# arnold117/PrimeKG-RGCN-LinkPrediction

Measured on AMD Instinct MI355X. Metric: edges/sec per RGCN layer (fwd+bwd), PrimeKG 30.9k nodes/849k edges/3 rels, higher is better.
Workload: dtype f32; 1 GPU; C2: PrimeKG-shaped synthetic graph, 30926 nodes / 849456 edge columns / 3 relations, encoder 64->128->128, 2 layers fwd+bwd, full graph per step, dropout 0; parallelism=1 GPU, launch=hipGraph replay

## Files before the change

### include/rgcn_hip.h

```cpp
#ifndef RGCN_HIP_H
#define RGCN_HIP_H

#include <stddef.h>
#include <stdint.h>

#ifdef __cplusplus
extern "C" {
#endif

#define RGCN_ABI_VERSION 27

enum {
  RGCN_OK = 0,
  RGCN_ERR_ARG = -1,
  RGCN_ERR_RANGE = -2,
  RGCN_ERR_HIP = -3,
  RGCN_ERR_UNSUPPORTED = -4,
  RGCN_ERR_WORKSPACE = -5
};

int rgcn_abi_version(void);
const char* rgcn_strerror(int code);

typedef struct rgcn_graph rgcn_graph;

int rgcn_graph_create(const int64_t* edge_index, const int64_t* edge_type, int64_t num_edges,
                      int64_t num_nodes, int64_t num_relations, void* stream,
                      rgcn_graph** out);
int rgcn_graph_create_bipartite(const int64_t* key_node, const int64_t* other_node,
                                const int64_t* edge_type, int64_t num_edges, int64_t num_key_nodes,
                                int64_t num_other_nodes, int64_t num_relations,
                                const float* edge_weight, void* stream, rgcn_graph** out);
void rgcn_graph_destroy(rgcn_graph* g);

int64_t rgcn_graph_num_edges(const rgcn_graph* g);
int64_t rgcn_graph_num_nodes(const rgcn_graph* g);
int64_t rgcn_graph_num_relations(const rgcn_graph* g);
float rgcn_graph_weight_bound(const rgcn_graph* g, int transposed);
int rgcn_graph_num_levels(const rgcn_graph* g, int transposed);

const uint32_t* rgcn_graph_tile_mask(const rgcn_graph* g, int transposed, int64_t* num_row_tiles);

int rgcn_graph_arrays(const rgcn_graph* g, int transposed, const int32_t** rowptr,
                      const int32_t** col, const int64_t** perm, const float** val);
int rgcn_graph_export(const rgcn_graph* g, int transposed, int32_t* rowptr, int32_t* col,
                      int64_t* perm, float* val, void* stream);

int rgcn_graph_import(int64_t num_edges, int64_t num_nodes, int64_t num_relations,
                      const int32_t* rowptr, const int32_t* col, const int64_t* perm, const float* cnt,
                      const int32_t* rowptr_t, const int32_t* col_t, const int64_t* perm_t,
                      const float* w_t, void* stream, rgcn_graph** out);

typedef struct rgcn_slab_job {
  const float* slab;
// ... 215 lines not shown
```

### primekg_rgcn_linkprediction_amd/_lib.py

```python
from __future__ import annotations

import ctypes
import os
from ctypes import c_float, POINTER, c_char_p, c_int, c_int64, c_size_t, c_void_p

import torch

ABI_VERSION = 27
LIB_NAME = "librgcn_hip.so"
LIB_PATH = os.path.join(os.path.dirname(os.path.abspath(__file__)), LIB_NAME)

RGCN_OK = 0
RGCN_ERR_ARG = -1
RGCN_ERR_RANGE = -2
RGCN_ERR_HIP = -3
RGCN_ERR_UNSUPPORTED = -4
RGCN_ERR_WORKSPACE = -5

_P = c_void_p
_I64 = c_int64

class SlabJob(ctypes.Structure):
    _fields_ = [("slab", c_void_p), ("bias_part", c_void_p), ("splits", ctypes.c_int32), ("K1", ctypes.c_int32),
                ("Kc", ctypes.c_int32), ("N", ctypes.c_int32), ("grad_weight", c_void_p), ("grad_root", c_void_p),
# ... 21 lines not shown
                                      7: (True, 0), 8: (True, 0), 9: (False, 0)},
}


PROTOTYPES = {
    "rgcn_abi_version": (c_int, []),
    "rgcn_strerror": (c_char_p, [c_int]),
    "rgcn_graph_create": (c_int, [_P, _P, _I64, _I64, _I64, _P, POINTER(c_void_p)]),
    "rgcn_graph_create_bipartite": (c_int, [_P, _P, _P, _I64, _I64, _I64, _I64, _P, _P, POINTER(c_void_p)]),
    "rgcn_graph_destroy": (None, [c_void_p]),
    "rgcn_graph_num_edges": (_I64, [c_void_p]),
    "rgcn_graph_num_nodes": (_I64, [c_void_p]),
    "rgcn_graph_num_relations": (_I64, [c_void_p]),
    "rgcn_graph_num_levels": (c_int, [c_void_p, c_int]),
    "rgcn_graph_weight_bound": (c_float, [c_void_p, c_int]),
    "rgcn_graph_arrays": (c_int, [c_void_p, c_int, POINTER(c_void_p), POINTER(c_void_p),
                                  POINTER(c_void_p), POINTER(c_void_p)]),
    "rgcn_graph_export": (c_int, [c_void_p, c_int, _P, _P, _P, _P, _P]),
    "rgcn_graph_import": (c_int, [_I64, _I64, _I64, _P, _P, _P, _P, _P, _P, _P, _P, _P, POINTER(c_void_p)]),
    "rgcn_aggregate_workspace_bytes": (c_size_t, [c_void_p, c_int, _I64]),
    "rgcn_aggregate": (c_int, [c_void_p, c_int, _P, _I64, _P, _P, c_size_t, _P]),
    "rgcn_aggregate_f16": (c_int, [c_void_p, c_int, _P, _I64, _P, _P, c_size_t, _P]),
    "rgcn_aggregate_level": (c_int, [c_void_p, c_int, c_int, _P, _I64, _P, _P, c_size_t, _P, _P]),
    "rgcn_graph_tile_mask": (c_void_p, [c_void_p, c_int, POINTER(c_int64)]),
    "rgcn_transform_fwd": (c_int, [_P, _P, _P, _P, _P, c_int, _P, _I64, _I64, _I64, _I64, _P, _P]),
    "rgcn_transform_fwd_f16_workspace_bytes": (c_size_t, [_I64, _I64, _I64]),
    "rgcn_transform_fwd_f16": (c_int, [_P, _P, _P, _P, _P, c_int, _P, _I64, _I64, _I64, _I64, _P, _P, c_size_t, _P]),
    "rgcn_transform_bwd_input": (c_int, [_P, _P, _P, _P, _P, _P, _I64, _I64, _I64, _I64, _P, _P]),
    "rgcn_transform_bwd_params_workspace_bytes": (c_size_t, [_I64, _I64, _I64, _I64]),
    "rgcn_transform_bwd_params": (c_int, [_P, _P, _P, _P, _I64, _I64, _I64, _I64, _P, _P, _P, _P,
# ... 116 lines not shown
```

### primekg_rgcn_linkprediction_amd/csrc/rgcn_aggregate.hip

```cpp
#include <algorithm>
#include <cstdlib>
#include <type_traits>

#include <hip/hip_fp16.h>

#include "rgcn_common.h"
#include "rgcn_slab_reduce.h"
#include "rgcn_hub_finish.h"

namespace {

constexpr int kThreads = 256;
constexpr int kUnroll = RGCN_HEAD;
#ifndef RGCN_REDUCE_UNROLL
#define RGCN_REDUCE_UNROLL 16
#endif

__device__ inline float4 f4zero() { return make_float4(0.f, 0.f, 0.f, 0.f); }
__device__ inline float f4amax(const float4& a) { return fmaxf(fmaxf(fabsf(a.x), fabsf(a.y)), fmaxf(fabsf(a.z), fabsf(a.w))); }

__device__ inline void f4add(float4& a, const float4& b) { a.x += b.x; a.y += b.y; a.z += b.z; a.w += b.w; }
__device__ inline void f4fma(float4& a, const float4& b, float s) {
  a.x = fmaf(b.x, s, a.x); a.y = fmaf(b.y, s, a.y); a.z = fmaf(b.z, s, a.z); a.w = fmaf(b.w, s, a.w);
}
// ... 29 lines not shown
    }
  }
  __device__ inline void advance(int gl, const int32_t* __restrict__ col, const float* __restrict__ w) {
    pos += RGCN_HEAD;
    if (pos == len) {
      cur = nxt;
      curw = nxtw;
      pos = 0;
      len = G;
      nbase += G;
      fetch_next(gl, col, w);
    }
  }
};

template <int G, bool WEIGHTED>
__device__ inline void aggregate_block(
    const int bx, float4* red, const float* __restrict__ src, const rgcn_item* __restrict__ items, int64_t nitems,
    const int32_t* __restrict__ col, const float* __restrict__ w, const float* __restrict__ cnt,
    float* __restrict__ agg, float* __restrict__ partial, int d, const int32_t* __restrict__ head_col,
    const float* __restrict__ head_w, unsigned* __restrict__ amax_out) {
  const int64_t item_id = ((int64_t)bx * kThreads + threadIdx.x) / G;
  const int c4 = ((int)threadIdx.x % G + (int)blockIdx.y * G) * 4;
  if (item_id >= nitems) return;
  const unsigned seen = rgcn_amax_peek(amax_out);
  const bool live = c4 < d;
  const rgcn_item it = items[item_id];
  const bool has_packs = (items[(int64_t)bx * (kThreads / G)].flags & RGCN_ITEM_PACK) != 0;

  float4 acc = f4zero();
  if constexpr (G >= RGCN_HEAD) {
    const int gl = (int)threadIdx.x % G;
    IdWindow<G, WEIGHTED> win;
    win.init(item_id, gl, it, col, w, head_col, head_w);
    for (int e = it.begin; e < it.end; e += kUnroll) {
      int idx[kUnroll];
      float wt[kUnroll];
      float4 v[kUnroll];
      win.get(idx, wt);
#pragma unroll
      for (int u = 0; u < kUnroll; ++u) {
        v[u] = f4zero();
        if (live && idx[u] >= 0) v[u] = *reinterpret_cast<const float4*>(src + (size_t)idx[u] * d + c4);
      }
      win.advance(gl, col, w);
#pragma unroll
      for (int u = 0; u < kUnroll; ++u) {
        if (WEIGHTED) f4fma(acc, v[u], wt[u]);
        else f4add(acc, v[u]);
      }
    }
  } else if (live) {
    int idx_n[kUnroll];
    float wt_n[kUnroll];
#pragma unroll
    for (int u = 0; u < kUnroll; ++u) {
      idx_n[u] = head_col[item_id * kUnroll + u];
      wt_n[u] = WEIGHTED ? head_w[item_id * kUnroll + u] : 0.f;
    }
    for (int e = it.begin; e < it.end; e += kUnroll) {
      int idx[kUnroll];
      float wt[kUnroll];
      float4 v[kUnroll];
#pragma unroll
      for (int u = 0; u < kUnroll; ++u) {
        idx[u] = idx_n[u];
        wt[u] = wt_n[u];
      }
#pragma unroll
      for (int u = 0; u < kUnroll; ++u) {
        v[u] = f4zero();
        if (idx[u] >= 0) v[u] = *reinterpret_cast<const float4*>(src + (size_t)idx[u] * d + c4);
      }
#pragma unroll
      for (int u = 0; u < kUnroll; ++u) {
        const int en = e + kUnroll + u;
        const bool ok = en < it.end;
        idx_n[u] = ok ? col[en] : -1;
        wt_n[u] = (WEIGHTED && ok) ? w[en] : 0.f;
      }
#pragma unroll
      for (int u = 0; u < kUnroll; ++u) {
        if (WEIGHTED) f4fma(acc, v[u], wt[u]);
        else f4add(acc, v[u]);
      }
    }
  }
  if (has_packs) {
    red[threadIdx.x] = acc;
    __syncthreads();
    if (it.flags & (RGCN_ITEM_MEMBER | RGCN_ITEM_SKIP)) return;
    const int followers = (it.flags >> RGCN_ITEM_FOLLOW_SHIFT) & (RGCN_PACK - 1);
    for (int f = 1; f <= followers; ++f) f4add(acc, red[threadIdx.x + f * G]);
  }
  if (!live) return;
  float lmax = 0.f;
  if (it.flags & RGCN_ITEM_FINAL) {
    if (cnt) {
      const float c = cnt[it.dst];
      acc.x /= c; acc.y /= c; acc.z /= c; acc.w /= c;
    }
    *reinterpret_cast<float4*>(agg + (size_t)it.dst * d + c4) = acc;
    lmax = f4amax(acc);
  } else {
    *reinterpret_cast<float4*>(partial + (size_t)it.dst * d + c4) = acc;
  }
  if (amax_out) rgcn_amax_publish(amax_out, lmax, seen);
}

template <int G, bool WEIGHTED>
__global__ __launch_bounds__(kThreads) void k_aggregate(
    const float* __restrict__ src, const rgcn_item* __restrict__ items, int64_t nitems,
    const int32_t* __restrict__ col, const float* __restrict__ w, const float* __restrict__ cnt,
    float* __restrict__ agg, float* __restrict__ partial, int d, const int32_t* __restrict__ head_col,
    const float* __restrict__ head_w, const rgcn_slab_job job, int gather_blocks, unsigned* __restrict__ amax_out) {
  __shared__ float4 red[kThreads];
  if ((int)blockIdx.x >= gather_blocks) {
    rgcn_slab_reduce_block<RGCN_SLAB_OUTS, RGCN_SLAB_GROUPS>(job, (int64_t)blockIdx.x - gather_blocks, red);
    return;
  }
  aggregate_block<G, WEIGHTED>((int)blockIdx.x, red, src, items, nitems, col, w, cnt, agg, partial, d, head_col, head_w, amax_out);
}

template <int G, bool WEIGHTED>
__global__ __launch_bounds__(kThreads) void k_aggregate_h(
    const __half* __restrict__ src, const rgcn_item* __restrict__ items, int64_t nitems,
    const int32_t* __restrict__ col, const float* __restrict__ w, const float* __restrict__ cnt,
    float* __restrict__ agg, float* __restrict__ partial, int d, const int32_t* __restrict__ head_col,
    const float* __restrict__ head_w) {
  const int64_t item_id = ((int64_t)blockIdx.x * kThreads + threadIdx.x) / G;
  __shared__ float4 red[2 * kThreads];
  const int c8 = ((int)threadIdx.x % G + (int)blockIdx.y * G) * 8;
  if (item_id >= nitems) return;
  const bool live = c8 < d;
  const rgcn_item it = items[item_id];
  const bool has_packs = (items[(int64_t)blockIdx.x * (kThreads / G)].flags & RGCN_ITEM_PACK) != 0;

  float acc[8];
#pragma unroll
  for (int k = 0; k < 8; ++k) acc[k] = 0.f;
  auto accumulate = [&](const uint4 (&v)[kUnroll], const float (&wt)[kUnroll]) {
#pragma unroll
    for (int u = 0; u < kUnroll; ++u) {
      const __half2* h2 = reinterpret_cast<const __half2*>(&v[u]);
#pragma unroll
      for (int k = 0; k < 4; ++k) {
        const float2 f = __half22float2(h2[k]);
        if (WEIGHTED) {
          acc[2 * k] = fmaf(f.x, wt[u], acc[2 * k]);
          acc[2 * k + 1] = fmaf(f.y, wt[u], acc[2 * k + 1]);
        } else {
// ... 79 lines not shown
template <int G>
__global__ __launch_bounds__(kThreads) void k_reduce_partials(const rgcn_item* __restrict__ items,
                                                              const float* __restrict__ cnt,
                                                              float* __restrict__ agg, float* partial, int d,
                                                              unsigned* __restrict__ amax_out) {
  __shared__ float4 red[kThreads];
  const float lmax = rgcn_reduce_item<G>(items[blockIdx.x], cnt, agg, partial, d, (int)blockIdx.y * G, red);
  if (amax_out && (int)threadIdx.x < G && (((int)threadIdx.x + (int)blockIdx.y * G) * 4 < d) &&
      (items[blockIdx.x].flags & RGCN_ITEM_FINAL))
    rgcn_amax_publish(amax_out, lmax);
}

template <int G>
void launch_level(const rgcn_csr* c, int level, bool weighted, const float* x, const float* cnt, float* agg,
                  float* partial, int d, hipStream_t stream, const rgcn_slab_job* tail = nullptr,
                  unsigned* amax_out = nullptr) {
  const int64_t nitems = c->num_items[level];
  if (nitems == 0) return;
  const unsigned gy = (unsigned)ceil_div64(d, 4 * G);
  if (level == 0) {
    const unsigned gather_blocks = (unsigned)ceil_div64(nitems, kThreads / G);
    const rgcn_slab_job job = tail ? *tail : rgcn_slab_job{};
    dim3 grid(gather_blocks + (tail ? (unsigned)rgcn_slab_reduce_blocks(job) : 0u), gy);
    if (weighted)
      k_aggregate<G, true><<<grid, kThreads, 0, stream>>>(x, c->items[0], nitems, c->col, c->val, cnt, agg, partial, d,
                                                          c->head_col, c->head_w, job, (int)gather_blocks, amax_out);
    else
      k_aggregate<G, false><<<grid, kThreads, 0, stream>>>(x, c->items[0], nitems, c->col, nullptr, cnt, agg, partial, d,
                                                           c->head_col, nullptr, job, (int)gather_blocks, amax_out);
  } else {
    dim3 grid((unsigned)nitems, gy);
    k_reduce_partials<G><<<grid, kThreads, 0, stream>>>(c->items[level], cnt, agg, partial, d, amax_out);
  }
}

template <int G>
void launch_level0_h(const rgcn_csr* c, bool weighted, const __half* x, const float* cnt, float* agg, float* partial,
                     int d, hipStream_t stream) {
  const int64_t nitems = c->num_items[0];
  if (nitems == 0) return;
  dim3 grid((unsigned)ceil_div64(nitems, kThreads / G), (unsigned)ceil_div64(d, 8 * G));
  if (weighted)
    k_aggregate_h<G, true><<<grid, kThreads, 0, stream>>>(x, c->items[0], nitems, c->col, c->val, cnt, agg, partial, d,
                                                            c->head_col, c->head_w);
  else
    k_aggregate_h<G, false><<<grid, kThreads, 0, stream>>>(x, c->items[0], nitems, c->col, nullptr, cnt, agg, partial, d,
                                                             c->head_col, nullptr);
}

int aggregate_levels(const rgcn_graph* g, int transposed, int first, int last, const float* x, int64_t d,
                     float* agg, void* workspace, size_t workspace_bytes, void* stream_, bool half_in = false,
                     const rgcn_slab_job* tail = nullptr, float* amax = nullptr) {
  if (!g || !agg || d <= 0 || (d & 3) || (half_in && (d & 7))) return RGCN_ERR_ARG;
  const rgcn_csr* c = &g->dir[transposed ? 1 : 0];
  if (!c->rowptr) return RGCN_ERR_ARG;
  if (c->n_key == 0) return RGCN_OK;
  if (!x) return RGCN_ERR_ARG;
  if (d > (1 << 20)) return RGCN_ERR_UNSUPPORTED;
  if (first < 0 || last > c->num_levels || first > last) return RGCN_ERR_ARG;
  if (c->num_partials > 0 &&
      (!workspace || workspace_bytes < (size_t)c->num_partials * (size_t)d * sizeof(float)))
    return RGCN_ERR_WORKSPACE;
// ... 1 lines not shown
  float* partial = (float*)workspace;
  unsigned* amax_out = reinterpret_cast<unsigned*>(amax);
  if (amax && half_in) return RGCN_ERR_UNSUPPORTED;
  const float* cnt = c->weighted ? nullptr : c->val;
  const bool weighted = c->weighted;
  const int q = (int)(d / 4);
  if (tail && tail->slab) {
    const bool can_ride = !half_in && first == 0 && last > 0 && d <= 256 && c->num_items[0] > 0;
    if (!can_ride) {
      k_slab_reduce<<<(unsigned)rgcn_slab_reduce_blocks(*tail), 256, 0, stream>>>(*tail);
      tail = nullptr;
    }
  } else {
    tail = nullptr;
  }
  for (int l = first; l < last; ++l) {
    const rgcn_slab_job* t0 = l == 0 ? tail : nullptr;
    if (l == 0 && half_in) {
      const __half* xh = reinterpret_cast<const __half*>(x);
      const int q8 = (int)(d / 8);
      if (q8 <= 1) launch_level0_h<1>(c, weighted, xh, cnt, agg, partial, (int)d, stream);
      else if (q8 <= 2) launch_level0_h<2>(c, weighted, xh, cnt, agg, partial, (int)d, stream);
      else if (q8 <= 4) launch_level0_h<4>(c, weighted, xh, cnt, agg, partial, (int)d, stream);
      else if (q8 <= 8) launch_level0_h<8>(c, weighted, xh, cnt, agg, partial, (int)d, stream);
      else if (q8 <= 16) launch_level0_h<16>(c, weighted, xh, cnt, agg, partial, (int)d, stream);
      else if (q8 <= 32) launch_level0_h<32>(c, weighted, xh, cnt, agg, partial, (int)d, stream);
      else launch_level0_h<64>(c, weighted, xh, cnt, agg, partial, (int)d, stream);
      continue;
    }
    if (q <= 1) launch_level<1>(c, l, weighted, x, cnt, agg, partial, (int)d, stream, t0, amax_out);
    else if (q <= 2) launch_level<2>(c, l, weighted, x, cnt, agg, partial, (int)d, stream, t0, amax_out);
    else if (q <= 4) launch_level<4>(c, l, weighted, x, cnt, agg, partial, (int)d, stream, t0, amax_out);
    else if (q <= 8) launch_level<8>(c, l, weighted, x, cnt, agg, partial, (int)d, stream, t0, amax_out);
    else if (q <= 16) launch_level<16>(c, l, weighted, x, cnt, agg, partial, (int)d, stream, t0, amax_out);
    else if (q <= 32) launch_level<32>(c, l, weighted, x, cnt, agg, partial, (int)d, stream, t0, amax_out);
    else launch_level<64>(c, l, weighted, x, cnt, agg, partial, (int)d, stream, t0, amax_out);
  }
  RGCN_HIP_TRY(hipGetLastError());
  return RGCN_OK;
}

}

extern "C" {

size_t rgcn_aggregate_workspace_bytes(const rgcn_graph* g, int transposed, int64_t d) {
  if (!g || d <= 0) return 0;
  return (size_t)g->dir[transposed ? 1 : 0].num_partials * (size_t)d * sizeof(float);
}

int rgcn_aggregate(const rgcn_graph* g, int transposed, const float* x, int64_t d, float* agg,
// ... 64 lines not shown
```

### primekg_rgcn_linkprediction_amd/csrc/rgcn_common.h

```cpp
#pragma once
#include <hip/hip_runtime.h>
#include <stdint.h>
#include "../../include/rgcn_hip.h"

#define RGCN_HIP_TRY(expr)                       \
  do {                                           \
    hipError_t err__ = (expr);                   \
    if (err__ != hipSuccess) return RGCN_ERR_HIP; \
  } while (0)

constexpr int RGCN_CHUNK = 64;
constexpr int RGCN_CHUNK_UP = 512;
constexpr int RGCN_MAX_LEVELS = 8;
constexpr int RGCN_HEAD = 8;

struct rgcn_item {
  int32_t begin, end, dst, flags;
};
constexpr int RGCN_PACK = 4;
enum : int32_t { RGCN_ITEM_FINAL = 1, RGCN_ITEM_PACK = 2, RGCN_ITEM_MEMBER = 4, RGCN_ITEM_SKIP = 8 };
constexpr int RGCN_ITEM_FOLLOW_SHIFT = 8;

struct rgcn_csr {
  int32_t* rowptr = nullptr;
// ... 1 lines not shown
  int64_t* perm = nullptr;
  float* val = nullptr;
  bool weighted = false;
  int64_t n_key = 0;
  int64_t n_other = 0;
  int num_levels = 0;
  rgcn_item* items[RGCN_MAX_LEVELS] = {};
  int64_t num_items[RGCN_MAX_LEVELS] = {};
  int64_t num_partials = 0;
  int32_t* head_col = nullptr;
  float* head_w = nullptr;
  uint32_t* tile_mask = nullptr;
  int64_t num_row_tiles = 0;
  int32_t* fin_ptr = nullptr;
  int64_t num_fin_tiles = 0;
  float weight_bound = 1.f;
};

struct rgcn_graph {
  int64_t E = 0, N = 0, R = 0;
  rgcn_csr dir[2];
};

static inline int64_t ceil_div64(int64_t a, int64_t b) { return (a + b - 1) / b; }

__attribute__((visibility("hidden"))) int* rgcn_index_error_flag();

constexpr int RGCN_AMAX_SLOTS = 64, RGCN_AMAX_STRIDE = 32;
constexpr int RGCN_AMAX_HEADS = 256, RGCN_AMAX_HEAD_STRIDE = 8;
static_assert(RGCN_AMAX_SLOTS * RGCN_AMAX_STRIDE == RGCN_AMAX_FLOATS, "amax buffer layout (include/rgcn_hip.h)");
static_assert(RGCN_AMAX_HEADS * RGCN_AMAX_HEAD_STRIDE == RGCN_AMAX_FLOATS && RGCN_AMAX_STRIDE % RGCN_AMAX_HEAD_STRIDE == 0,
// ... 36 lines not shown
```

### primekg_rgcn_linkprediction_amd/csrc/rgcn_graph.hip

```cpp
#include <hipcub/hipcub.hpp>

#include <algorithm>
#include <cmath>
#include <new>
#include <vector>

#include "rgcn_common.h"

namespace {

constexpr int kThreads = 256;

__global__ void k_validate(const int64_t* __restrict__ key_node, const int64_t* __restrict__ other_node,
                           const int64_t* __restrict__ edge_type, int64_t E, int64_t n_key, int64_t n_other,
                           int64_t R, int* __restrict__ flag) {
  int64_t e = (int64_t)blockIdx.x * blockDim.x + threadIdx.x;
  if (e >= E) return;
  int64_t k = key_node[e], o = other_node[e], t = edge_type[e];
  if (k < 0 || k >= n_key || o < 0 || o >= n_other || t < 0 || t >= R) atomicOr(flag, 1);
}

__global__ void k_make_keys(const int64_t* __restrict__ key_node, const int64_t* __restrict__ edge_type,
                            int64_t E, int64_t R, uint32_t* __restrict__ keys, uint32_t* __restrict__ ids) {
  int64_t e = (int64_t)blockIdx.x * blockDim.x + threadIdx.x;
// ... 33 lines not shown
                               float* __restrict__ w) {
  int64_t e = (int64_t)blockIdx.x * blockDim.x + threadIdx.x;
  if (e >= E) return;
  int64_t rel = (int64_t)(skeys_t[e] % (uint32_t)R);
  w[e] = 1.0f / cnt[(int64_t)col_t[e] * R + rel];
}

__global__ void k_permute_weights(const float* __restrict__ w_in, const int64_t* __restrict__ perm, int64_t E,
                                  float* __restrict__ w) {
  int64_t e = (int64_t)blockIdx.x * blockDim.x + threadIdx.x;
  if (e < E) w[e] = w_in[perm[e]];
}

inline unsigned grid_for(int64_t n) { return (unsigned)std::max<int64_t>(1, ceil_div64(n, kThreads)); }

int build_plan(const std::vector<int32_t>& rowptr, int64_t NR, int64_t R, rgcn_csr* csr) {
  struct Pending { int32_t seg, begin, end; };
  struct Pack { int32_t begin, end, dst, final_row; };
  std::vector<std::vector<rgcn_item>> levels;
  std::vector<Pending> pending, next;
  std::vector<rgcn_item> singles;
  std::vector<Pack> packs;
  int64_t partial_rows = 0;

  for (int64_t s = 0; s < NR; ++s) {
    const int32_t begin = rowptr[s], end = rowptr[s + 1], len = end - begin;
    if (len <= RGCN_CHUNK) {
      singles.push_back({begin, end, (int32_t)s, RGCN_ITEM_FINAL});
      continue;
    }
    const int32_t span = RGCN_CHUNK * RGCN_PACK;
    const int32_t npacks = (int32_t)ceil_div64(len, span);
    if (npacks == 1) {
      packs.push_back({begin, end, (int32_t)s, 1});
    } else {
      const int32_t pbase = (int32_t)partial_rows;
      for (int32_t p = 0; p < npacks; ++p)
        packs.push_back({begin + p * span, std::min(begin + (p + 1) * span, end), pbase + p, 0});
      partial_rows += npacks;
      pending.push_back({(int32_t)s, pbase, pbase + npacks});
    }
// ... 41 lines not shown
    partial_rows += nch;
    nxt.push_back({p.seg, pbase, pbase + nch});
  };
  while (!pending.empty()) {
    if ((int)levels.size() >= RGCN_MAX_LEVELS) return RGCN_ERR_UNSUPPORTED;
    levels.emplace_back();
    next.clear();
    for (const Pending& p : pending) emit_up(levels.back(), next, p);
    std::stable_sort(levels.back().begin(), levels.back().end(), [](const rgcn_item& a, const rgcn_item& b) {
      return (a.end - a.begin) > (b.end - b.begin);
    });
    pending.swap(next);
  }
  if (partial_rows > INT32_MAX) return RGCN_ERR_UNSUPPORTED;

  std::vector<int32_t> fin_ptr;
  if (levels.size() == 2 && !levels[1].empty() && R > 0) {
    const int64_t tiles = ceil_div64(csr->n_key, 32);
    auto tile_of = [&](const rgcn_item& it) { return (int64_t)(it.dst / R) >> 5; };
    std::stable_sort(levels[1].begin(), levels[1].end(),
                     [&](const rgcn_item& a, const rgcn_item& b) { return tile_of(a) < tile_of(b); });
    fin_ptr.assign((size_t)tiles + 1, 0);
    for (const rgcn_item& it : levels[1]) ++fin_ptr[(size_t)tile_of(it) + 1];
    for (int64_t t = 0; t < tiles; ++t) fin_ptr[(size_t)t + 1] += fin_ptr[(size_t)t];
  }

  csr->num_levels = (int)levels.size();
  csr->num_partials = partial_rows;
  for (int l = 0; l < csr->num_levels; ++l) {
    auto& v = levels[l];
    csr->num_items[l] = (int64_t)v.size();
    if (v.empty()) continue;
    RGCN_HIP_TRY(hipMalloc((void**)&csr->items[l], v.size() * sizeof(rgcn_item)));
    RGCN_HIP_TRY(hipMemcpy(csr->items[l], v.data(), v.size() * sizeof(rgcn_item), hipMemcpyHostToDevice));
  }
  if (!fin_ptr.empty()) {
    RGCN_HIP_TRY(hipMalloc((void**)&csr->fin_ptr, fin_ptr.size() * sizeof(int32_t)));
    RGCN_HIP_TRY(hipMemcpy(csr->fin_ptr, fin_ptr.data(), fin_ptr.size() * sizeof(int32_t), hipMemcpyHostToDevice));
    csr->num_fin_tiles = (int64_t)fin_ptr.size() - 1;
  }
  return RGCN_OK;
}

void free_csr(rgcn_csr* c) {
  (void)hipFree(c->rowptr);
  (void)hipFree(c->col);
  (void)hipFree(c->perm);
  (void)hipFree(c->val);
  (void)hipFree(c->tile_mask);
  (void)hipFree(c->fin_ptr);
  (void)hipFree(c->head_col);
  (void)hipFree(c->head_w);
  for (int l = 0; l < RGCN_MAX_LEVELS; ++l) (void)hipFree(c->items[l]);
  *c = rgcn_csr();
}

struct Scratch {
  uint32_t *keys = nullptr, *ids = nullptr, *skeys[2] = {nullptr, nullptr}, *sids = nullptr;
  void* sort_tmp = nullptr;
  size_t sort_tmp_bytes = 0;
  int* flag = nullptr;
  int alloc(int64_t E) {
    RGCN_HIP_TRY(hipMalloc((void**)&flag, sizeof(int)));
    if (E <= 0) return RGCN_OK;
    RGCN_HIP_TRY(hipMalloc((void**)&keys, E * sizeof(uint32_t)));
// ... 302 lines not shown
  if (!g) return;
  free_csr(&g->dir[0]);
  free_csr(&g->dir[1]);
  delete g;
}

int64_t rgcn_graph_num_edges(const rgcn_graph* g) { return g ? g->E : -1; }
int64_t rgcn_graph_num_nodes(const rgcn_graph* g) { return g ? g->N : -1; }
int64_t rgcn_graph_num_relations(const rgcn_graph* g) { return g ? g->R : -1; }
float rgcn_graph_weight_bound(const rgcn_graph* g, int transposed) {
  if (!g) return 0.f;
  const rgcn_csr* c = &g->dir[transposed ? 1 : 0];
  return c->rowptr ? c->weight_bound : 0.f;
}

int rgcn_graph_num_levels(const rgcn_graph* g, int transposed) {
  return g ? g->dir[transposed ? 1 : 0].num_levels : -1;
}

const uint32_t* rgcn_graph_tile_mask(const rgcn_graph* g, int transposed, int64_t* num_row_tiles) {
  if (!g) return nullptr;
  const rgcn_csr* c = &g->dir[transposed ? 1 : 0];
  if (num_row_tiles) *num_row_tiles = c->num_row_tiles;
  return c->tile_mask;
}

int rgcn_graph_arrays(const rgcn_graph* g, int transposed, const int32_t** rowptr, const int32_t** col,
                      const int64_t** perm, const float** val) {
  if (!g) return RGCN_ERR_ARG;
  const rgcn_csr* c = &g->dir[transposed ? 1 : 0];
// ... 24 lines not shown
```

### primekg_rgcn_linkprediction_amd/csrc/rgcn_hub_finish.h

```cpp
#pragma once
#include "rgcn_common.h"

#ifndef RGCN_REDUCE_UNROLL
#define RGCN_REDUCE_UNROLL 16
#endif

#if defined(__HIPCC__)
template <int G>
__device__ inline float rgcn_reduce_item(const rgcn_item it, const float* __restrict__ cnt, float* __restrict__ agg,
                                         float* partial, int d, int col0, float4* red) {
  constexpr int SLOTS = 256 / G;
  const int gl = (int)threadIdx.x % G, slot = (int)threadIdx.x / G;
  const int c4 = (gl + col0) * 4;
  const bool live = c4 < d;
  float4 acc = make_float4(0.f, 0.f, 0.f, 0.f);
  if (live) {
    for (int r0 = it.begin + slot; r0 < it.end; r0 += SLOTS * RGCN_REDUCE_UNROLL) {
      float4 v[RGCN_REDUCE_UNROLL];
#pragma unroll
      for (int u = 0; u < RGCN_REDUCE_UNROLL; ++u) {
        const int row = r0 + u * SLOTS;
        v[u] = make_float4(0.f, 0.f, 0.f, 0.f);
        if (row < it.end) v[u] = *reinterpret_cast<const float4*>(partial + (size_t)row * d + c4);
      }
#pragma unroll
      for (int u = 0; u < RGCN_REDUCE_UNROLL; ++u) {
        acc.x += v[u].x; acc.y += v[u].y; acc.z += v[u].z; acc.w += v[u].w;
      }
    }
  }
  red[threadIdx.x] = acc;
  __syncthreads();
  float lmax = 0.f;
  if (slot == 0 && live) {
    float4 s = red[gl];
#pragma unroll
    for (int k = 1; k < SLOTS; ++k) {
      const float4 t = red[k * G + gl];
      s.x += t.x; s.y += t.y; s.z += t.z; s.w += t.w;
    }
    if (it.flags & RGCN_ITEM_FINAL) {
// ... 14 lines not shown
```

Before: 6.262 billion edges/s.

## Finish hub reductions in-kernel via tickets and fold zero-row clearing into gather

Level-0 gather blocks that write hub partial rows now take an atomic ticket per hub. The last contributor does the level-1 reduction inside the same kernel, so the separate reduce-partials launch goes away when there are exactly two levels. Destination rows with no edges are listed at plan time and zeroed by extra blocks in the gather kernel, instead of by a separate clear. This relies on write-through stores, agent-scope fences and a ticket reset, which adds synchronisation overhead and memory-ordering risk.

```diff
diff --git a/include/rgcn_hip.h b/include/rgcn_hip.h
--- a/include/rgcn_hip.h
+++ b/include/rgcn_hip.h
@@ -8,7 +8,7 @@
 extern "C" {
 #endif
 
-#define RGCN_ABI_VERSION 27
+#define RGCN_ABI_VERSION 28
 
 enum {
   RGCN_OK = 0,
@@ -38,6 +38,11 @@
 int64_t rgcn_graph_num_relations(const rgcn_graph* g);
 float rgcn_graph_weight_bound(const rgcn_graph* g, int transposed);
 int rgcn_graph_num_levels(const rgcn_graph* g, int transposed);
+int rgcn_plan_hubs(const int32_t* rowptr, int64_t num_keys, int64_t num_relations, int32_t* owner,
+                   int64_t owner_capacity, int64_t* num_partials, int32_t* hubs, int64_t hubs_capacity,
+                   int64_t* num_hubs, int* num_levels);
+int64_t rgcn_plan_zero_keys(const int32_t* rowptr, int64_t num_keys, int64_t num_relations, int32_t* keys,
+                            int64_t capacity);
 
 const uint32_t* rgcn_graph_tile_mask(const rgcn_graph* g, int transposed, int64_t* num_row_tiles);
 
diff --git a/primekg_rgcn_linkprediction_amd/_lib.py b/primekg_rgcn_linkprediction_amd/_lib.py
--- a/primekg_rgcn_linkprediction_amd/_lib.py
+++ b/primekg_rgcn_linkprediction_amd/_lib.py
@@ -6,7 +6,7 @@
 
 import torch
 
-ABI_VERSION = 27
+ABI_VERSION = 28
 LIB_NAME = "librgcn_hip.so"
 LIB_PATH = os.path.join(os.path.dirname(os.path.abspath(__file__)), LIB_NAME)
 
@@ -59,6 +59,8 @@
     "rgcn_graph_num_relations": (_I64, [c_void_p]),
     "rgcn_graph_num_levels": (c_int, [c_void_p, c_int]),
     "rgcn_graph_weight_bound": (c_float, [c_void_p, c_int]),
+    "rgcn_plan_zero_keys": (_I64, [_P, _I64, _I64, _P, _I64]),
+    "rgcn_plan_hubs": (c_int, [_P, _I64, _I64, _P, _I64, POINTER(c_int64), _P, _I64, POINTER(c_int64), POINTER(c_int)]),
     "rgcn_graph_arrays": (c_int, [c_void_p, c_int, POINTER(c_void_p), POINTER(c_void_p),
                                   POINTER(c_void_p), POINTER(c_void_p)]),
     "rgcn_graph_export": (c_int, [c_void_p, c_int, _P, _P, _P, _P, _P]),
diff --git a/primekg_rgcn_linkprediction_amd/csrc/rgcn_aggregate.hip b/primekg_rgcn_linkprediction_amd/csrc/rgcn_aggregate.hip
--- a/primekg_rgcn_linkprediction_amd/csrc/rgcn_aggregate.hip
+++ b/primekg_rgcn_linkprediction_amd/csrc/rgcn_aggregate.hip
@@ -67,54 +67,69 @@
   }
 };
 
+typedef float rgcn_f32x4 __attribute__((ext_vector_type(4)));
+__device__ inline void store_row_through(float* p, const float4& a) {
+  const rgcn_f32x4 v = {a.x, a.y, a.z, a.w};
+  asm volatile("global_store_dwordx4 %0, %1, off sc1\n\ts_nop 1" : : "v"(p), "v"(v) : "memory");
+}
+
+constexpr int kNoteF4 = 1 + kThreads / RGCN_PACK / 4;
+constexpr int kFinUnroll = 8;
+
 template <int G, bool WEIGHTED>
 __device__ inline void aggregate_block(
     const int bx, float4* red, const float* __restrict__ src, const rgcn_item* __restrict__ items, int64_t nitems,
     const int32_t* __restrict__ col, const float* __restrict__ w, const float* __restrict__ cnt,
-    float* __restrict__ agg, float* __restrict__ partial, int d, const int32_t* __restrict__ head_col,
-    const float* __restrict__ head_w, unsigned* __restrict__ amax_out) {
+    float* __restrict__ agg, float* partial, int d, const int32_t* __restrict__ head_col,
+    const float* __restrict__ head_w, unsigned* __restrict__ amax_out, const rgcn_hub_fin fin) {
   const int64_t item_id = ((int64_t)bx * kThreads + threadIdx.x) / G;
   const int c4 = ((int)threadIdx.x % G + (int)blockIdx.y * G) * 4;
-  if (item_id >= nitems) return;
+  const bool has_packs = (items[(int64_t)bx * (kThreads / G)].flags & RGCN_ITEM_PACK) != 0;
+  const bool valid = item_id < nitems;
+  if (!valid) {
+    if (!has_packs) return;
+  }
   const unsigned seen = rgcn_amax_peek(amax_out);
   const bool live = c4 < d;
-  const rgcn_item it = items[item_id];
-  const bool has_packs = (items[(int64_t)bx * (kThreads / G)].flags & RGCN_ITEM_PACK) != 0;
+  rgcn_item it = {0, 0, 0, RGCN_ITEM_PACK | RGCN_ITEM_SKIP};
+  if (valid) it = items[item_id];
 
   float4 acc = f4zero();
   if constexpr (G >= RGCN_HEAD) {
-    const int gl = (int)threadIdx.x % G;
-    IdWindow<G, WEIGHTED> win;
-    win.init(item_id, gl, it, col, w, head_col, head_w);
+    if (valid) {
+      const int gl = (int)threadIdx.x % G;
+      IdWindow<G, WEIGHTED> win;
+      win.init(item_id, gl, it, col, w, head_col, head_w);
+      for (int e = it.begin; e < it.end; e += kUnroll) {
+        int idx[kUnroll];
+        float wt[kUnroll];
+        float4 v[kUnroll];
+        win.get(idx, wt);
+#pragma unroll
+        for (int u = 0; u < kUnroll; ++u) {
+          v[u] = f4zero();
+          if (live && idx[u] >= 0) v[u] = *reinterpret_cast<const float4*>(src + (size_t)idx[u] * d + c4);
+        }
+        win.advance(gl, col, w);
+#pragma unroll
+        for (int u = 0; u < kUnroll; ++u) {
+          if (WEIGHTED) f4fma(acc, v[u], wt[u]);
+          else f4add(acc, v[u]);
+        }
+      }
+    }
+  } else if (live && valid) {
+    int idx_n[kUnroll];
+    float wt_n[kUnroll];
+#pragma unroll
+    for (int u = 0; u < kUnroll; ++u) {
+      idx_n[u] = head_col[item_id * kUnroll + u];
+      wt_n[u] = WEIGHTED ? head_w[item_id * kUnroll + u] : 0.f;
+    }
     for (int e = it.begin; e < it.end; e += kUnroll) {
       int idx[kUnroll];
       float wt[kUnroll];
       float4 v[kUnroll];
-      win.get(idx, wt);
-#pragma unroll
-      for (int u = 0; u < kUnroll; ++u) {
-        v[u] = f4zero();
-        if (live && idx[u] >= 0) v[u] = *reinterpret_cast<const float4*>(src + (size_t)idx[u] * d + c4);
-      }
-      win.advance(gl, col, w);
-#pragma unroll
-      for (int u = 0; u < kUnroll; ++u) {
-        if (WEIGHTED) f4fma(acc, v[u], wt[u]);
-        else f4add(acc, v[u]);
-      }
-    }
-  } else if (live) {
-    int idx_n[kUnroll];
-    float wt_n[kUnroll];
-#pragma unroll
-    for (int u = 0; u < kUnroll; ++u) {
-      idx_n[u] = head_col[item_id * kUnroll + u];
-      wt_n[u] = WEIGHTED ? head_w[item_id * kUnroll + u] : 0.f;
-    }
-    for (int e = it.begin; e < it.end; e += kUnroll) {
-      int idx[kUnroll];
-      float wt[kUnroll];
-      float4 v[kUnroll];
 #pragma unroll
       for (int u = 0; u < kUnroll; ++u) {
         idx[u] = idx_n[u];
@@ -139,40 +154,127 @@
       }
     }
   }
+  const bool hub_lead = fin.owner != nullptr &&
+                        (it.flags & (RGCN_ITEM_PACK | RGCN_ITEM_MEMBER | RGCN_ITEM_SKIP | RGCN_ITEM_FINAL)) == RGCN_ITEM_PACK;
+  bool hub_here = false;
+  int* note = reinterpret_cast<int*>(red + kThreads);
   if (has_packs) {
     red[threadIdx.x] = acc;
+    if (fin.owner != nullptr) {
+      const bool any = __any(hub_lead) != 0;
+      if ((threadIdx.x & 63) == 0) note[threadIdx.x >> 6] = any ? 1 : 0;
+    }
     __syncthreads();
-    if (it.flags & (RGCN_ITEM_MEMBER | RGCN_ITEM_SKIP)) return;
-    const int followers = (it.flags >> RGCN_ITEM_FOLLOW_SHIFT) & (RGCN_PACK - 1);
-    for (int f = 1; f <= followers; ++f) f4add(acc, red[threadIdx.x + f * G]);
-  }
-  if (!live) return;
-  float lmax = 0.f;
-  if (it.flags & RGCN_ITEM_FINAL) {
-    if (cnt) {
-      const float c = cnt[it.dst];
-      acc.x /= c; acc.y /= c; acc.z /= c; acc.w /= c;
-    }
-    *reinterpret_cast<float4*>(agg + (size_t)it.dst * d + c4) = acc;
-    lmax = f4amax(acc);
-  } else {
-    *reinterpret_cast<float4*>(partial + (size_t)it.dst * d + c4) = acc;
-  }
-  if (amax_out) rgcn_amax_publish(amax_out, lmax, seen);
-}
+    if (fin.owner != nullptr) hub_here = (note[0] | note[1] | note[2] | note[3]) != 0;
+    const bool writer = !(it.flags & (RGCN_ITEM_MEMBER | RGCN_ITEM_SKIP));
+    if (!writer) {
+      if (!hub_here) return;
+    } else {
+      const int followers = (it.flags >> RGCN_ITEM_FOLLOW_SHIFT) & (RGCN_PACK - 1);
+      for (int f = 1; f <= followers; ++f) f4add(acc, red[threadIdx.x + f * G]);
+    }
+  }
+  if (!live) {
+    if (!hub_here) return;
+  }
+  if (live && !(it.flags & (RGCN_ITEM_MEMBER | RGCN_ITEM_SKIP))) {
+    float lmax = 0.f;
+    if (it.flags & RGCN_ITEM_FINAL) {
+      if (cnt) {
+        const float c = cnt[it.dst];
+        acc.x /= c; acc.y /= c; acc.z /= c; acc.w /= c;
+      }
+      *reinterpret_cast<float4*>(agg + (size_t)it.dst * d + c4) = acc;
+      lmax = f4amax(acc);
+    } else if (hub_lead) {
+      store_row_through(partial + (size_t)it.dst * d + c4, acc);
+    } else {
+      *reinterpret_cast<float4*>(partial + (size_t)it.dst * d + c4) = acc;
+    }
+    if (amax_out) rgcn_amax_publish(amax_out, lmax, seen);
+  }
+  if (!hub_here) return;
+
+  const int gl = (int)threadIdx.x % G, slot = (int)threadIdx.x / G;
+  const bool drawer = hub_lead && gl == 0;
+  int own = 0;
+  rgcn_item up = {0, 0, 0, 0};
+  if (drawer) {
+    own = fin.owner[it.dst];
+    up = fin.items1[own];
+  }
+  asm volatile("s_waitcnt vmcnt(0)" ::: "memory");
+  __syncthreads();
+  if (gl == 0 && slot % RGCN_PACK == 0) {
+    int mine = 0;
+    if (drawer) {
+      const unsigned t = __hip_atomic_fetch_add(fin.ticket + own, 1u, __ATOMIC_RELAXED, __HIP_MEMORY_SCOPE_AGENT);
+      if (t + 1u == (unsigned)(up.end - up.begin)) {
+        __hip_atomic_store(fin.ticket + own, 0u, __ATOMIC_RELAXED, __HIP_MEMORY_SCOPE_AGENT);
+        mine = own + 1;
+      }
+    }
+    note[4 + slot / RGCN_PACK] = mine;
+  }
+  __syncthreads();
+  constexpr int kPacks = kThreads / G / RGCN_PACK;
+  bool acquired = false;
+  for (int p = 0; p < kPacks; ++p) {
+    const int o = note[4 + p];
+    if (o == 0) continue;
+    if (!acquired && threadIdx.x == 0) {
+      __builtin_amdgcn_fence(__ATOMIC_ACQUIRE, "agent");
+      asm volatile("s_waitcnt vmcnt(0)" ::: "memory");
+    }
+    acquired = true;
+    __syncthreads();
+    const float m = rgcn_reduce_item<G, kFinUnroll>(fin.items1[o - 1], cnt, agg, partial, d, 0, red);
+    if (amax_out && (int)threadIdx.x < G && (int)threadIdx.x * 4 < d) rgcn_amax_publish(amax_out, m);
+  }
+}
+
+constexpr int kZeroRows = 8;
+template <int G, int F4>
+__device__ inline void zero_rows_block(const int rb, const rgcn_zero_job zero, float* __restrict__ agg, int d) {
+  constexpr int kSlots = kThreads / G;
+  const int c = ((int)threadIdx.x % G + (int)blockIdx.y * G) * 4 * F4;
+  const int64_t base = ((int64_t)rb * kZeroRows) * kSlots + (int)threadIdx.x / G;
+  int key[kZeroRows];
+#pragma unroll
+  for (int u = 0; u < kZeroRows; ++u) {
+    const int64_t i = base + (int64_t)u * kSlots;
+    key[u] = i < zero.count ? zero.key[i] : -1;
+  }
+  if (c >= d) return;
+#pragma unroll
+  for (int u = 0; u < kZeroRows; ++u) {
+    if (key[u] < 0) continue;
+    float4* row = reinterpret_cast<float4*>(agg + (size_t)key[u] * d + c);
+#pragma unroll
+    for (int f = 0; f < F4; ++f) row[f] = f4zero();
+  }
+}
+template <int G>
+inline int zero_rows_blocks(const rgcn_csr* c) { return (int)ceil_div64(c->num_zero, (kThreads / G) * kZeroRows); }
 
 template <int G, bool WEIGHTED>
 __global__ __launch_bounds__(kThreads) void k_aggregate(
     const float* __restrict__ src, const rgcn_item* __restrict__ items, int64_t nitems,
     const int32_t* __restrict__ col, const float* __restrict__ w, const float* __restrict__ cnt,
-    float* __restrict__ agg, float* __restrict__ partial, int d, const int32_t* __restrict__ head_col,
-    const float* __restrict__ head_w, const rgcn_slab_job job, int gather_blocks, unsigned* __restrict__ amax_out) {
-  __shared__ float4 red[kThreads];
-  if ((int)blockIdx.x >= gather_blocks) {
-    rgcn_slab_reduce_block<RGCN_SLAB_OUTS, RGCN_SLAB_GROUPS>(job, (int64_t)blockIdx.x - gather_blocks, red);
+    float* __restrict__ agg, float* partial, int d, const int32_t* __restrict__ head_col,
+    const float* __restrict__ head_w, const rgcn_slab_job job, int gather_blocks, unsigned* __restrict__ amax_out,
+    const rgcn_hub_fin fin, const rgcn_zero_job zero) {
+  __shared__ float4 red[kThreads + kNoteF4];
+  if ((int)blockIdx.x < zero.blocks) {
+    zero_rows_block<G, 1>((int)blockIdx.x, zero, agg, d);
     return;
   }
-  aggregate_block<G, WEIGHTED>((int)blockIdx.x, red, src, items, nitems, col, w, cnt, agg, partial, d, head_col, head_w, amax_out);
+  const int bx = (int)blockIdx.x - zero.blocks;
+  if (bx >= gather_blocks) {
+    rgcn_slab_reduce_block<RGCN_SLAB_OUTS, RGCN_SLAB_GROUPS>(job, (int64_t)bx - gather_blocks, red);
+    return;
+  }
+  aggregate_block<G, WEIGHTED>(bx, red, src, items, nitems, col, w, cnt, agg, partial, d, head_col, head_w, amax_out, fin);
 }
 
 template <int G, bool WEIGHTED>
@@ -180,14 +282,19 @@
     const __half* __restrict__ src, const rgcn_item* __restrict__ items, int64_t nitems,
     const int32_t* __restrict__ col, const float* __restrict__ w, const float* __restrict__ cnt,
     float* __restrict__ agg, float* __restrict__ partial, int d, const int32_t* __restrict__ head_col,
-    const float* __restrict__ head_w) {
-  const int64_t item_id = ((int64_t)blockIdx.x * kThreads + threadIdx.x) / G;
+    const float* __restrict__ head_w, const rgcn_zero_job zero) {
+  if ((int)blockIdx.x < zero.blocks) {
+    zero_rows_block<G, 2>((int)blockIdx.x, zero, agg, d);
+    return;
+  }
+  const int bx = (int)blockIdx.x - zero.blocks;
+  const int64_t item_id = ((int64_t)bx * kThreads + threadIdx.x) / G;
   __shared__ float4 red[2 * kThreads];
   const int c8 = ((int)threadIdx.x % G + (int)blockIdx.y * G) * 8;
   if (item_id >= nitems) return;
   const bool live = c8 < d;
   const rgcn_item it = items[item_id];
-  const bool has_packs = (items[(int64_t)blockIdx.x * (kThreads / G)].flags & RGCN_ITEM_PACK) != 0;
+  const bool has_packs = (items[(int64_t)bx * (kThreads / G)].flags & RGCN_ITEM_PACK) != 0;
 
   float acc[8];
 #pragma unroll
@@ -297,20 +404,23 @@
 template <int G>
 void launch_level(const rgcn_csr* c, int level, bool weighted, const float* x, const float* cnt, float* agg,
                   float* partial, int d, hipStream_t stream, const rgcn_slab_job* tail = nullptr,
-                  unsigned* amax_out = nullptr) {
+                  unsigned* amax_out = nullptr, bool finish_hubs = false) {
   const int64_t nitems = c->num_items[level];
-  if (nitems == 0) return;
+  if (nitems == 0 && (level > 0 || c->num_zero == 0)) return;
   const unsigned gy = (unsigned)ceil_div64(d, 4 * G);
   if (level == 0) {
     const unsigned gather_blocks = (unsigned)ceil_div64(nitems, kThreads / G);
     const rgcn_slab_job job = tail ? *tail : rgcn_slab_job{};
-    dim3 grid(gather_blocks + (tail ? (unsigned)rgcn_slab_reduce_blocks(job) : 0u), gy);
+    const rgcn_zero_job zero{c->zero_key, c->num_zero, zero_rows_blocks<G>(c)};
+    dim3 grid((unsigned)zero.blocks + gather_blocks + (tail ? (unsigned)rgcn_slab_reduce_blocks(job) : 0u), gy);
+    rgcn_hub_fin fin;
+    if (finish_hubs) fin = rgcn_hub_fin{c->items[1], c->hub_owner, c->hub_ticket};
     if (weighted)
       k_aggregate<G, true><<<grid, kThreads, 0, stream>>>(x, c->items[0], nitems, c->col, c->val, cnt, agg, partial, d,
-                                                          c->head_col, c->head_w, job, (int)gather_blocks, amax_out);
+                                                          c->head_col, c->head_w, job, (int)gather_blocks, amax_out, fin, zero);
     else
       k_aggregate<G, false><<<grid, kThreads, 0, stream>>>(x, c->items[0], nitems, c->col, nullptr, cnt, agg, partial, d,
-                                                           c->head_col, nullptr, job, (int)gather_blocks, amax_out);
+                                                           c->head_col, nullptr, job, (int)gather_blocks, amax_out, fin, zero);
   } else {
     dim3 grid((unsigned)nitems, gy);
     k_reduce_partials<G><<<grid, kThreads, 0, stream>>>(c->items[level], cnt, agg, partial, d, amax_out);
@@ -321,14 +431,15 @@
 void launch_level0_h(const rgcn_csr* c, bool weighted, const __half* x, const float* cnt, float* agg, float* partial,
                      int d, hipStream_t stream) {
   const int64_t nitems = c->num_items[0];
-  if (nitems == 0) return;
-  dim3 grid((unsigned)ceil_div64(nitems, kThreads / G), (unsigned)ceil_div64(d, 8 * G));
+  if (nitems == 0 && c->num_zero == 0) return;
+  const rgcn_zero_job zero{c->zero_key, c->num_zero, zero_rows_blocks<G>(c)};
+  dim3 grid((unsigned)zero.blocks + (unsigned)ceil_div64(nitems, kThreads / G), (unsigned)ceil_div64(d, 8 * G));
   if (weighted)
     k_aggregate_h<G, true><<<grid, kThreads, 0, stream>>>(x, c->items[0], nitems, c->col, c->val, cnt, agg, partial, d,
-                                                            c->head_col, c->head_w);
+                                                            c->head_col, c->head_w, zero);
   else
     k_aggregate_h<G, false><<<grid, kThreads, 0, stream>>>(x, c->items[0], nitems, c->col, nullptr, cnt, agg, partial, d,
-                                                             c->head_col, nullptr);
+                                                             c->head_col, nullptr, zero);
 }
 
 int aggregate_levels(const rgcn_graph* g, int transposed, int first, int last, const float* x, int64_t d,
@@ -360,6 +471,8 @@
   } else {
     tail = nullptr;
   }
+  const bool finish_hubs = !half_in && first == 0 && last == 2 && c->num_levels == 2 && c->hub_owner && d <= 256;
+  if (finish_hubs) last = 1;
   for (int l = first; l < last; ++l) {
     const rgcn_slab_job* t0 = l == 0 ? tail : nullptr;
     if (l == 0 && half_in) {
@@ -374,13 +487,13 @@
       else launch_level0_h<64>(c, weighted, xh, cnt, agg, partial, (int)d, stream);
       continue;
     }
-    if (q <= 1) launch_level<1>(c, l, weighted, x, cnt, agg, partial, (int)d, stream, t0, amax_out);
-    else if (q <= 2) launch_level<2>(c, l, weighted, x, cnt, agg, partial, (int)d, stream, t0, amax_out);
-    else if (q <= 4) launch_level<4>(c, l, weighted, x, cnt, agg, partial, (int)d, stream, t0, amax_out);
-    else if (q <= 8) launch_level<8>(c, l, weighted, x, cnt, agg, partial, (int)d, stream, t0, amax_out);
-    else if (q <= 16) launch_level<16>(c, l, weighted, x, cnt, agg, partial, (int)d, stream, t0, amax_out);
-    else if (q <= 32) launch_level<32>(c, l, weighted, x, cnt, agg, partial, (int)d, stream, t0, amax_out);
-    else launch_level<64>(c, l, weighted, x, cnt, agg, partial, (int)d, stream, t0, amax_out);
+    if (q <= 1) launch_level<1>(c, l, weighted, x, cnt, agg, partial, (int)d, stream, t0, amax_out, finish_hubs);
+    else if (q <= 2) launch_level<2>(c, l, weighted, x, cnt, agg, partial, (int)d, stream, t0, amax_out, finish_hubs);
+    else if (q <= 4) launch_level<4>(c, l, weighted, x, cnt, agg, partial, (int)d, stream, t0, amax_out, finish_hubs);
+    else if (q <= 8) launch_level<8>(c, l, weighted, x, cnt, agg, partial, (int)d, stream, t0, amax_out, finish_hubs);
+    else if (q <= 16) launch_level<16>(c, l, weighted, x, cnt, agg, partial, (int)d, stream, t0, amax_out, finish_hubs);
+    else if (q <= 32) launch_level<32>(c, l, weighted, x, cnt, agg, partial, (int)d, stream, t0, amax_out, finish_hubs);
+    else launch_level<64>(c, l, weighted, x, cnt, agg, partial, (int)d, stream, t0, amax_out, finish_hubs);
   }
   RGCN_HIP_TRY(hipGetLastError());
   return RGCN_OK;
diff --git a/primekg_rgcn_linkprediction_amd/csrc/rgcn_common.h b/primekg_rgcn_linkprediction_amd/csrc/rgcn_common.h
--- a/primekg_rgcn_linkprediction_amd/csrc/rgcn_common.h
+++ b/primekg_rgcn_linkprediction_amd/csrc/rgcn_common.h
@@ -39,7 +39,23 @@
   int64_t num_row_tiles = 0;
   int32_t* fin_ptr = nullptr;
   int64_t num_fin_tiles = 0;
+  int32_t* hub_owner = nullptr;
+  unsigned* hub_ticket = nullptr;
+  int32_t* zero_key = nullptr;
+  int64_t num_zero = 0;
   float weight_bound = 1.f;
+};
+
+struct rgcn_hub_fin {
+  const rgcn_item* items1 = nullptr;
+  const int32_t* owner = nullptr;
+  unsigned* ticket = nullptr;
+};
+
+struct rgcn_zero_job {
+  const int32_t* key = nullptr;
+  int64_t count = 0;
+  int blocks = 0;
 };
 
 struct rgcn_graph {
diff --git a/primekg_rgcn_linkprediction_amd/csrc/rgcn_graph.hip b/primekg_rgcn_linkprediction_amd/csrc/rgcn_graph.hip
--- a/primekg_rgcn_linkprediction_amd/csrc/rgcn_graph.hip
+++ b/primekg_rgcn_linkprediction_amd/csrc/rgcn_graph.hip
@@ -71,10 +71,16 @@
 
 inline unsigned grid_for(int64_t n) { return (unsigned)std::max<int64_t>(1, ceil_div64(n, kThreads)); }
 
-int build_plan(const std::vector<int32_t>& rowptr, int64_t NR, int64_t R, rgcn_csr* csr) {
+struct HostPlan {
+  std::vector<std::vector<rgcn_item>> levels;
+  int64_t partial_rows = 0;
+  std::vector<int32_t> fin_ptr, hub_owner, zero_key;
+};
+
+int plan_host(const int32_t* rowptr, int64_t NR, int64_t R, int64_t n_key, HostPlan* out) {
   struct Pending { int32_t seg, begin, end; };
   struct Pack { int32_t begin, end, dst, final_row; };
-  std::vector<std::vector<rgcn_item>> levels;
+  std::vector<std::vector<rgcn_item>>& levels = out->levels;
   std::vector<Pending> pending, next;
   std::vector<rgcn_item> singles;
   std::vector<Pack> packs;
@@ -82,6 +88,10 @@
 
   for (int64_t s = 0; s < NR; ++s) {
     const int32_t begin = rowptr[s], end = rowptr[s + 1], len = end - begin;
+    if (len == 0) {
+      out->zero_key.push_back((int32_t)s);
+      continue;
+    }
     if (len <= RGCN_CHUNK) {
       singles.push_back({begin, end, (int32_t)s, RGCN_ITEM_FINAL});
       continue;
@@ -153,9 +163,9 @@
   }
   if (partial_rows > INT32_MAX) return RGCN_ERR_UNSUPPORTED;
 
-  std::vector<int32_t> fin_ptr;
+  std::vector<int32_t>& fin_ptr = out->fin_ptr;
   if (levels.size() == 2 && !levels[1].empty() && R > 0) {
-    const int64_t tiles = ceil_div64(csr->n_key, 32);
+    const int64_t tiles = ceil_div64(n_key, 32);
     auto tile_of = [&](const rgcn_item& it) { return (int64_t)(it.dst / R) >> 5; };
     std::stable_sort(levels[1].begin(), levels[1].end(),
                      [&](const rgcn_item& a, const rgcn_item& b) { return tile_of(a) < tile_of(b); });
@@ -163,9 +173,24 @@
     for (const rgcn_item& it : levels[1]) ++fin_ptr[(size_t)tile_of(it) + 1];
     for (int64_t t = 0; t < tiles; ++t) fin_ptr[(size_t)t + 1] += fin_ptr[(size_t)t];
   }
-
+  std::vector<int32_t>& hub_owner = out->hub_owner;
+  if (levels.size() == 2 && !levels[1].empty()) {
+    hub_owner.assign((size_t)partial_rows, -1);
+    for (size_t i = 0; i < levels[1].size(); ++i)
+      for (int32_t p = levels[1][i].begin; p < levels[1][i].end; ++p) hub_owner[(size_t)p] = (int32_t)i;
+  }
+  out->partial_rows = partial_rows;
+  return RGCN_OK;
+}
+
+int build_plan(const std::vector<int32_t>& rowptr, int64_t NR, int64_t R, rgcn_csr* csr) {
+  HostPlan plan;
+  const int rc = plan_host(rowptr.data(), NR, R, csr->n_key, &plan);
+  if (rc != RGCN_OK) return rc;
+  std::vector<std::vector<rgcn_item>>& levels = plan.levels;
+  const std::vector<int32_t>&fin_ptr = plan.fin_ptr, &hub_owner = plan.hub_owner;
   csr->num_levels = (int)levels.size();
-  csr->num_partials = partial_rows;
+  csr->num_partials = plan.partial_rows;
   for (int l = 0; l < csr->num_levels; ++l) {
     auto& v = levels[l];
     csr->num_items[l] = (int64_t)v.size();
@@ -177,6 +202,17 @@
     RGCN_HIP_TRY(hipMalloc((void**)&csr->fin_ptr, fin_ptr.size() * sizeof(int32_t)));
     RGCN_HIP_TRY(hipMemcpy(csr->fin_ptr, fin_ptr.data(), fin_ptr.size() * sizeof(int32_t), hipMemcpyHostToDevice));
     csr->num_fin_tiles = (int64_t)fin_ptr.size() - 1;
+  }
+  csr->num_zero = (int64_t)plan.zero_key.size();
+  if (csr->num_zero > 0) {
+    RGCN_HIP_TRY(hipMalloc((void**)&csr->zero_key, plan.zero_key.size() * sizeof(int32_t)));
+    RGCN_HIP_TRY(hipMemcpy(csr->zero_key, plan.zero_key.data(), plan.zero_key.size() * sizeof(int32_t), hipMemcpyHostToDevice));
+  }
+  if (!hub_owner.empty()) {
+    RGCN_HIP_TRY(hipMalloc((void**)&csr->hub_owner, hub_owner.size() * sizeof(int32_t)));
+    RGCN_HIP_TRY(hipMemcpy(csr->hub_owner, hub_owner.data(), hub_owner.size() * sizeof(int32_t), hipMemcpyHostToDevice));
+    RGCN_HIP_TRY(hipMalloc((void**)&csr->hub_ticket, levels[1].size() * sizeof(unsigned)));
+    RGCN_HIP_TRY(hipMemset(csr->hub_ticket, 0, levels[1].size() * sizeof(unsigned)));
   }
   return RGCN_OK;
 }
@@ -188,6 +224,9 @@
   (void)hipFree(c->val);
   (void)hipFree(c->tile_mask);
   (void)hipFree(c->fin_ptr);
+  (void)hipFree(c->hub_owner);
+  (void)hipFree(c->hub_ticket);
+  (void)hipFree(c->zero_key);
   (void)hipFree(c->head_col);
   (void)hipFree(c->head_w);
   for (int l = 0; l < RGCN_MAX_LEVELS; ++l) (void)hipFree(c->items[l]);
@@ -520,6 +559,42 @@
   return c->rowptr ? c->weight_bound : 0.f;
 }
 
+int rgcn_plan_hubs(const int32_t* rowptr, int64_t num_keys, int64_t num_relations, int32_t* owner,
+                   int64_t owner_capacity, int64_t* num_partials, int32_t* hubs, int64_t hubs_capacity,
+                   int64_t* num_hubs, int* num_levels) {
+  if (!rowptr || num_keys < 0 || num_relations <= 0 || owner_capacity < 0 || hubs_capacity < 0) return RGCN_ERR_ARG;
+  if (too_big(num_keys, 0, num_relations, 0)) return RGCN_ERR_UNSUPPORTED;
+  HostPlan plan;
+  const int rc = plan_host(rowptr, num_keys * num_relations, num_relations, num_keys, &plan);
+  if (rc != RGCN_OK) return rc;
+  const bool one = plan.levels.size() == 2;
+  const int64_t np = one ? (int64_t)plan.hub_owner.size() : 0, nh = one ? (int64_t)plan.levels[1].size() : 0;
+  if (num_levels) *num_levels = (int)plan.levels.size();
+  if (num_partials) *num_partials = np;
+  if (num_hubs) *num_hubs = nh;
+  if (owner)
+    for (int64_t p = 0; p < std::min(np, owner_capacity); ++p) owner[p] = plan.hub_owner[(size_t)p];
+  if (hubs)
+    for (int64_t i = 0; i < std::min(nh, hubs_capacity); ++i) {
+      const rgcn_item& it = plan.levels[1][(size_t)i];
+      hubs[3 * i] = it.begin; hubs[3 * i + 1] = it.end; hubs[3 * i + 2] = it.dst;
+    }
+  return RGCN_OK;
+}
+
+int64_t rgcn_plan_zero_keys(const int32_t* rowptr, int64_t num_keys, int64_t num_relations, int32_t* keys,
+                            int64_t capacity) {
+  if (!rowptr || num_keys < 0 || num_relations <= 0 || capacity < 0) return RGCN_ERR_ARG;
+  if (too_big(num_keys, 0, num_relations, 0)) return RGCN_ERR_UNSUPPORTED;
+  HostPlan plan;
+  const int rc = plan_host(rowptr, num_keys * num_relations, num_relations, num_keys, &plan);
+  if (rc != RGCN_OK) return rc;
+  const int64_t n = (int64_t)plan.zero_key.size();
+  if (keys)
+    for (int64_t i = 0; i < std::min(n, capacity); ++i) keys[i] = plan.zero_key[(size_t)i];
+  return n;
+}
+
 int rgcn_graph_num_levels(const rgcn_graph* g, int transposed) {
   return g ? g->dir[transposed ? 1 : 0].num_levels : -1;
 }
diff --git a/primekg_rgcn_linkprediction_amd/csrc/rgcn_hub_finish.h b/primekg_rgcn_linkprediction_amd/csrc/rgcn_hub_finish.h
--- a/primekg_rgcn_linkprediction_amd/csrc/rgcn_hub_finish.h
+++ b/primekg_rgcn_linkprediction_amd/csrc/rgcn_hub_finish.h
@@ -6,7 +6,7 @@
 #endif
 
 #if defined(__HIPCC__)
-template <int G>
+template <int G, int UNROLL = RGCN_REDUCE_UNROLL>
 __device__ inline float rgcn_reduce_item(const rgcn_item it, const float* __restrict__ cnt, float* __restrict__ agg,
                                          float* partial, int d, int col0, float4* red) {
   constexpr int SLOTS = 256 / G;
@@ -15,16 +15,16 @@
   const bool live = c4 < d;
   float4 acc = make_float4(0.f, 0.f, 0.f, 0.f);
   if (live) {
-    for (int r0 = it.begin + slot; r0 < it.end; r0 += SLOTS * RGCN_REDUCE_UNROLL) {
-      float4 v[RGCN_REDUCE_UNROLL];
+    for (int r0 = it.begin + slot; r0 < it.end; r0 += SLOTS * UNROLL) {
+      float4 v[UNROLL];
 #pragma unroll
-      for (int u = 0; u < RGCN_REDUCE_UNROLL; ++u) {
+      for (int u = 0; u < UNROLL; ++u) {
         const int row = r0 + u * SLOTS;
         v[u] = make_float4(0.f, 0.f, 0.f, 0.f);
         if (row < it.end) v[u] = *reinterpret_cast<const float4*>(partial + (size_t)row * d + c4);
       }
 #pragma unroll
-      for (int u = 0; u < RGCN_REDUCE_UNROLL; ++u) {
+      for (int u = 0; u < UNROLL; ++u) {
         acc.x += v[u].x; acc.y += v[u].y; acc.z += v[u].z; acc.w += v[u].w;
       }
     }
```

Measured after the change: 6.526 billion edges/s, median of 6. 4.2% higher.
